# swiss-territorial-data-lab/proj-roadsurf

Hardware: AMD Instinct MI355X
Metric: tiles_per_sec_512x512x3 (higher is better)
Workload: dtype f16 hi + lo operand planes (22 significand bits, 3 MFMA products per product) / f32 accumulate; 1 GPU; Mask R-CNN R50-FPN inference, batch 16 of 512x512 3-band tiles per GPU (BASELINE configs[1]), 800x800 network input; seeded synthetic weights, saturated: 1000 proposals and 100 detections per tile; batch_per_gpu=16, lanes=2, lane_streams=independent, num_classes=2, weights=random

## Files before the change

proj_roadsurf_amd/csrc/bneck_split.hip:

```cpp
#include "conv_tile.h"

namespace {

constexpr int NJ = 2, NT = 256, BM = 4 * NJ * 16, PXW = NJ * 16;

template <int CB, bool PROJ = false>
struct SCfg {
  static constexpr int CBW = 64 * CB;
  static constexpr int C4 = 256 * CB;
  static constexpr int MIB = 4 * CB;
  static constexpr int NPASS = 4 * CB;
  static constexpr int KS2 = 9 * 2 * CB;
  static constexpr int STAGE = (BM + CBW) * 128;
  static constexpr int S3 = 2 * CB + (PROJ ? 2 : 0);
  static constexpr int W3K = CBW + (PROJ ? 64 : 0);
  static constexpr int W3_BYTES = S3 * 64 * 128;
  static constexpr int W1_BYTES = 2 * CBW * 128;
  static constexpr int PASS_BYTES = W3_BYTES + W1_BYTES;
  static constexpr int LDS_BYTES = 2 * STAGE > PASS_BYTES ? 2 * STAGE : PASS_BYTES;
};

__device__ __forceinline__ void split8(const f32x4& a, const f32x4& b, half8& h, half8& l) {
#pragma unroll
  for (int r = 0; r < 4; ++r) {
    const HiLo sa = split_round(a[r]), sb = split_round(b[r]);
    h[r] = sa.h; l[r] = sa.l;
    h[4 + r] = sb.h; l[4 + r] = sb.l;
  }
}
__device__ __forceinline__ float relu_clamp(float v, unsigned& satc, bool count) {
  v = v > 0.f ? v : 0.f;
  satc += count ? rs_sat_bad(v) : 0u;
  return clamp_h16_pos(v);
}

template <int CB, bool NEXT, bool PROJ>
__global__ __launch_bounds__(NT, 2) void bneck_tail_split_kernel(const BneckSplitParams p) {
  using G = SCfg<CB, PROJ>;
  static_assert(!PROJ || CB == 1, "projection form: 64-wide stage only");
  constexpr int CBW = G::CBW, C4 = G::C4, MIB = G::MIB, NPASS = G::NPASS, KS2 = G::KS2, STAGE = G::STAGE;
  extern __shared__ __attribute__((aligned(16))) char smem[];
  const int tid = threadIdx.x, lane = tid & 63;
  const int wave = __builtin_amdgcn_readfirstlane(tid >> 6);
  const int M = p.M;
  const int ntiles = (M + BM - 1) / BM;
  const int q = blockIdx.x;
  if (q >= ntiles) return;
  const int m0 = xcd_tile(q, ntiles) * BM;
  const int lrow = lane >> 3, lchk = lane & 7;
  const half_t* aptr[BM / 32];
#pragma unroll
  for (int ps = 0; ps < BM / 32; ++ps) {
    int m = m0 + ps * 32 + wave * 8 + lrow;
    if (m >= M) m = M - 1;
    const Pix px = pix_of(m, p.W, p.H);
    aptr[ps] = p.t1 + ((long long)(px.n * p.Hp + px.y) * p.Wp + px.x) * CBW + chunk_split(src_chunk(lchk, act_key(lrow)), p.t1_lo);
  }
  const half_t* wptr[CBW / 32];
#pragma unroll
  for (int ps = 0; ps < CBW / 32; ++ps) {
    const int row = ps * 32 + wave * 8 + lrow;
    wptr[ps] = p.w2 + (long long)row * (9 * CBW) + chunk_split(src_chunk(lchk, w_key(row, 4 * MIB)), p.w2_lo);
  }
  auto stage_tap = [&](int buf, int step) {
    char* abase = smem + buf * STAGE;
    const int slice = step / 9, tap = step - slice * 9;
    const int a_off = ((tap / 3) * p.Wp + (tap % 3)) * CBW + slice * 32;
#pragma unroll
    for (int ps = 0; ps < BM / 32; ++ps) glds16(aptr[ps] + a_off, abase + (ps * 32 + wave * 8) * 128);
#pragma unroll
    for (int ps = 0; ps < CBW / 32; ++ps) glds16(wptr[ps] + tap * CBW + slice * 32, abase + BM * 128 + (ps * 32 + wave * 8) * 128);
  };
  auto stage_pass = [&](int pass) {
#pragma unroll
    for (int ps = 0; ps < 2; ++ps) {
      const int row = ps * 32 + wave * 8 + lrow;
      const long long dch = chunk_split(src_chunk(lchk, w_key(row, 16)), p.w3_lo);
#pragma unroll
      for (int s = 0; s < G::S3; ++s)
        glds16(p.w3p + (long long)(pass * 64 + row) * G::W3K + s * 32 + dch, smem + s * 8192 + (ps * 32 + wave * 8) * 128);
    }
    if (NEXT) {
#pragma unroll
      for (int ps = 0; ps < CBW / 32; ++ps) {
        const int row = ps * 32 + wave * 8 + lrow;
        const long long dch = chunk_split(src_chunk(lchk, w_key(row, 4 * MIB)), p.w1_lo);
#pragma unroll
        for (int s = 0; s < 2; ++s)
          glds16(p.w1p + (long long)row * C4 + pass * 64 + s * 32 + dch, smem + G::W3_BYTES + s * CBW * 128 + (ps * 32 + wave * 8) * 128);
      }
    }
  };

  const int fi = lane & 15, fq = lane >> 4, fkey = lane & 7;
  int w_off[4], wB_off[MIB], x_off[NJ];
#pragma unroll
  for (int i = 0; i < 4; ++i) w_off[i] = frag_row(fi, i, 16) * 128;
#pragma unroll
  for (int i = 0; i < MIB; ++i) wB_off[i] = frag_row(fi, i, 4 * MIB) * 128;
#pragma unroll
  for (int j = 0; j < NJ; ++j) x_off[j] = (wave * PXW + j * 16 + fi) * 128;
  const int ch_off = frag_off(fq, fkey, 0), cl_off = frag_off(fq, fkey, 1);

  long long opix[NJ];
  bool valid[NJ];
  unsigned satc = 0;
#pragma unroll
  for (int j = 0; j < NJ; ++j) {
    const int m = m0 + wave * PXW + j * 16 + fi;
    valid[j] = m < M;
    const int mm = valid[j] ? m : M - 1;
    const Pix px = pix_of(mm, p.W, p.H);
    opix[j] = (long long)(px.n * p.Hp + px.y + 1) * p.Wp + px.x + 1;
  }

  f32x4 acc[MIB][NJ];
#pragma unroll
  for (int i = 0; i < MIB; ++i)
#pragma unroll
    for (int j = 0; j < NJ; ++j) acc[i][j] = f32x4{0.f, 0.f, 0.f, 0.f};
  stage_tap(0, 0);
  auto stage_x0 = [&](char* base) {
#pragma unroll
    for (int ps = 0; ps < BM / 32; ++ps) {
      int m = m0 + ps * 32 + wave * 8 + lrow;
      if (m >= M) m = M - 1;
      const Pix px = pix_of(m, p.W, p.H);
      const half_t* xp = p.x0 + ((long long)(px.n * p.Hp + px.y + 1) * p.Wp + px.x + 1) * 64 + chunk_split(src_chunk(lchk, act_key(lrow)), p.x0_lo);
#pragma unroll
      for (int s = 0; s < 2; ++s) glds16(xp + s * 32, base + s * BM * 128 + (ps * 32 + wave * 8) * 128);
    }
  };
  for (int t = 0; t < KS2; ++t) {
    asm volatile("s_waitcnt vmcnt(0)" ::: "memory");
    __syncthreads();
    if (t + 1 < KS2) stage_tap((t + 1) & 1, t + 1);
    const char* sb = smem + (t & 1) * STAGE;
    half8 xh[NJ], xl[NJ];
#pragma unroll
    for (int j = 0; j < NJ; ++j) { xh[j] = *(const half8*)(sb + x_off[j] + ch_off); xl[j] = *(const half8*)(sb + x_off[j] + cl_off); }
#pragma unroll
    for (int i = 0; i < MIB; ++i) {
      const half8 wh = *(const half8*)(sb + BM * 128 + wB_off[i] + ch_off), wl = *(const half8*)(sb + BM * 128 + wB_off[i] + cl_off);
#pragma unroll
      for (int j = 0; j < NJ; ++j) mfma_split3(acc[i][j], wh, wl, xh[j], xl[j]);
    }
  }
  half8 th[2 * CB][NJ], tl[2 * CB][NJ];
  {
#pragma unroll
    for (int i = 0; i < MIB; ++i) {
      const f32x4 sc = *(const f32x4*)(p.s2 + fq * 4 * MIB + i * 4), bv = *(const f32x4*)(p.b2 + fq * 4 * MIB + i * 4);
#pragma unroll
      for (int j = 0; j < NJ; ++j)
#pragma unroll
        for (int r = 0; r < 4; ++r) acc[i][j][r] = relu_clamp(acc[i][j][r] * sc[r] + bv[r], satc, valid[j]);
    }
#pragma unroll
    for (int s = 0; s < 2 * CB; ++s)
#pragma unroll
      for (int j = 0; j < NJ; ++j) split8(acc[2 * s][j], acc[2 * s + 1][j], th[s][j], tl[s][j]);
  }
  half8 x0h[PROJ ? 2 : 1][NJ], x0l[PROJ ? 2 : 1][NJ];
  if (PROJ) {
    const char* xb = smem;
    __syncthreads();
    stage_x0(smem);
    asm volatile("s_waitcnt vmcnt(0)" ::: "memory");
    __syncthreads();
#pragma unroll
    for (int s = 0; s < 2; ++s)
#pragma unroll
      for (int j = 0; j < NJ; ++j) {
        x0h[s][j] = *(const half8*)(xb + s * BM * 128 + x_off[j] + ch_off);
        x0l[s][j] = *(const half8*)(xb + s * BM * 128 + x_off[j] + cl_off);
      }
  }
  f32x4 acc3[MIB][NJ];
#pragma unroll
  for (int i = 0; i < MIB; ++i)
#pragma unroll
    for (int j = 0; j < NJ; ++j) acc3[i][j] = f32x4{0.f, 0.f, 0.f, 0.f};

  for (int pass = 0; pass < NPASS; ++pass) {
    __syncthreads();
    stage_pass(pass);
    const int cb = pass * 64 + fq * 16;
    half8 rh[NJ][2], rl[NJ][2];
    if (!PROJ) {
#pragma unroll
      for (int j = 0; j < NJ; ++j) {
        const half_t* xp = p.x + opix[j] * C4 + cb;
        rh[j][0] = *(const half8*)xp; rh[j][1] = *(const half8*)(xp + 8);
        rl[j][0] = *(const half8*)(xp + p.x_lo); rl[j][1] = *(const half8*)(xp + p.x_lo + 8);
      }
    }
    asm volatile("s_waitcnt vmcnt(0)" ::: "memory");
    __syncthreads();
#pragma unroll
    for (int j = 0; j < NJ; ++j) {
      f32x4 a2[4];
#pragma unroll
      for (int i = 0; i < 4; ++i) {
        a2[i] = f32x4{0.f, 0.f, 0.f, 0.f};
#pragma unroll
        for (int s = 0; s < 2 * CB; ++s) {
          const half8 wh = *(const half8*)(smem + s * 8192 + w_off[i] + ch_off), wl = *(const half8*)(smem + s * 8192 + w_off[i] + cl_off);
          mfma_split3(a2[i], wh, wl, th[s][j], tl[s][j]);
        }
        if (PROJ) {
#pragma unroll
          for (int s = 0; s < 2; ++s) {
            const half8 wh = *(const half8*)(smem + (2 * CB + s) * 8192 + w_off[i] + ch_off), wl = *(const half8*)(smem + (2 * CB + s) * 8192 + w_off[i] + cl_off);
            mfma_split3(a2[i], wh, wl, x0h[s][j], x0l[s][j]);
          }
        }
      }
#pragma unroll
      for (int i = 0; i < 4; ++i) {
        const f32x4 s3v = *(const f32x4*)(p.s3 + cb + i * 4), b3v = *(const f32x4*)(p.b3 + cb + i * 4);
#pragma unroll
        for (int r = 0; r < 4; ++r) {
          const float res = PROJ ? 0.f : (float)rh[j][i >> 1][(i & 1) * 4 + r] + (float)rl[j][i >> 1][(i & 1) * 4 + r];
          a2[i][r] = relu_clamp(a2[i][r] * s3v[r] + b3v[r] + res, satc, valid[j]);
        }
      }
      half8 o0h, o0l, o1h, o1l;
      split8(a2[0], a2[1], o0h, o0l);
      split8(a2[2], a2[3], o1h, o1l);
      if (valid[j]) {
        half_t* op = p.out + opix[j] * C4 + cb;
        *(half8*)op = o0h; *(half8*)(op + 8) = o1h;
        *(half8*)(op + p.out_lo) = o0l; *(half8*)(op + p.out_lo + 8) = o1l;
      }
      if (NEXT) {
#pragma unroll
        for (int i = 0; i < MIB; ++i) {
          const char* wb = smem + G::W3_BYTES + wB_off[i];
          const half8 w0h = *(const half8*)(wb + ch_off), w0l = *(const half8*)(wb + cl_off);
          const half8 w1h = *(const half8*)(wb + CBW * 128 + ch_off), w1l = *(const half8*)(wb + CBW * 128 + cl_off);
          mfma_split3(acc3[i][j], w0h, w0l, o0h, o0l);
          mfma_split3(acc3[i][j], w1h, w1l, o1h, o1l);
        }
      }
    }
  }
  if (NEXT) {
#pragma unroll
    for (int j = 0; j < NJ; ++j) {
      if (!valid[j]) continue;
      half_t* op = p.t1n + opix[j] * CBW + fq * 4 * MIB;
#pragma unroll
      for (int k = 0; k < MIB / 2; ++k) {
        const f32x4 sa = *(const f32x4*)(p.s1 + fq * 4 * MIB + 8 * k), sb2 = *(const f32x4*)(p.s1 + fq * 4 * MIB + 8 * k + 4);
        const f32x4 ba = *(const f32x4*)(p.b1 + fq * 4 * MIB + 8 * k), bb = *(const f32x4*)(p.b1 + fq * 4 * MIB + 8 * k + 4);
        f32x4 va, vb;
#pragma unroll
        for (int r = 0; r < 4; ++r) { va[r] = relu_clamp(acc3[2 * k][j][r] * sa[r] + ba[r], satc, true); vb[r] = relu_clamp(acc3[2 * k + 1][j][r] * sb2[r] + bb[r], satc, true); }
        half8 h, l;
        split8(va, vb, h, l);
        *(half8*)(op + 8 * k) = h;
        *(half8*)(op + p.t1n_lo + 8 * k) = l;
      }
    }
  }
  rs_sat_flush(p.sat, satc);
}

template <int CB, bool PROJ>
int launch_split_cb(const BneckSplitParams& p, hipStream_t stream) {
  using G = SCfg<CB, PROJ>;
  const long long nblk = cdiv(p.M, BM);
  RS_CHECK(nblk < (1ll << 31), RS_ERR_ARG, "bneck_tail_split: grid too large");
  const void* k = p.w1p ? (const void*)bneck_tail_split_kernel<CB, true, PROJ> : (const void*)bneck_tail_split_kernel<CB, false, PROJ>;
  static bool attr[2] = {false, false};
  const int ai = p.w1p ? 1 : 0;
  if (!attr[ai]) {
    RS_HIP(hipFuncSetAttribute(k, hipFuncAttributeMaxDynamicSharedMemorySize, G::LDS_BYTES));
    attr[ai] = true;
  }
  BneckSplitParams pc = p;
  void* args[] = {&pc};
  RS_HIP(hipLaunchKernel(k, dim3((unsigned)nblk), dim3(NT), args, G::LDS_BYTES, stream));
  return RS_OK;
}

}

int launch_bneck_tail_split(const BneckSplitParams& p, hipStream_t stream) {
  RS_CHECK(p.M > 0 && p.t1 && p.w2 && p.b2 && p.s2 && p.w3p && p.b3 && p.s3 && (p.x || p.x0) && !(p.x && p.x0) && p.out, RS_ERR_ARG, "bneck_tail_split: null argument");
  RS_CHECK(p.Hp == p.H + 2 && p.Wp == p.W + 2, RS_ERR_ARG, "bneck_tail_split: maps must carry a halo of 1");
  RS_CHECK(!p.w1p || (p.b1 && p.s1 && p.t1n), RS_ERR_ARG, "bneck_tail_split: next conv1 needs weights, scales, bias and output");
  RS_CHECK(p.CB == 1 || p.CB == 2, RS_ERR_UNSUPPORTED, "bneck_tail_split: bottleneck width %d (64 or 128)", 64 * p.CB);
  if (p.x0) {
    RS_CHECK(p.CB == 1, RS_ERR_UNSUPPORTED, "bneck_tail_split: the projection-shortcut form exists for the 64-wide stage only");
    return launch_split_cb<1, true>(p, stream);
  }
  return p.CB == 1 ? launch_split_cb<1, false>(p, stream) : launch_split_cb<2, false>(p, stream);
}
```

proj_roadsurf_amd/csrc/common.h:

```cpp
#pragma once
#include <hip/hip_runtime.h>
#include <stdint.h>
#include <stdio.h>

typedef _Float16 half_t;
typedef _Float16 half4 __attribute__((ext_vector_type(4)));
typedef _Float16 half8 __attribute__((ext_vector_type(8)));
typedef float f32x4 __attribute__((ext_vector_type(4)));

#define RS_OK 0
#define RS_ERR_ARG -1
#define RS_ERR_HIP -2
#define RS_ERR_BLOB -3
#define RS_ERR_UNSUPPORTED -4

void rs_set_error(const char* fmt, ...);

#define RS_HIP(expr)                                                                       \
  do {                                                                                     \
    hipError_t _e = (expr);                                                                \
    if (_e != hipSuccess) {                                                                \
      rs_set_error("%s:%d: %s -> %s", __FILE__, __LINE__, #expr, hipGetErrorString(_e));   \
      return RS_ERR_HIP;                                                                   \
    }                                                                                      \
  } while (0)

#define RS_CHECK(cond, code, ...)  \
  do {                             \
    if (!(cond)) {                 \
      rs_set_error(__VA_ARGS__);   \
      return (code);               \
    }                              \
  } while (0)

static inline int cdiv(long long a, long long b) { return (int)((a + b - 1) / b); }

#if defined(__HIPCC__)
__device__ __forceinline__ float rs_fdiv(float a, float b) {
  const float y0 = __builtin_amdgcn_rcpf(b);
  const float e = __builtin_fmaf(-b, y0, 1.0f);
  const float y = __builtin_fmaf(e, y0, y0);
  const float q0 = a * y;
  const float r0 = __builtin_fmaf(-b, q0, a);
  const float q1 = __builtin_fmaf(r0, y, q0);
  const float r1 = __builtin_fmaf(-b, q1, a);
  const float q = __builtin_fmaf(r1, y, q1);
  const bool special = !(__builtin_fabsf(b) > 0.f && __builtin_fabsf(b) < __builtin_inff() && __builtin_fabsf(a) > 0.f && __builtin_fabsf(a) < __builtin_inff());
  return special ? a * y0 : q;
}

__device__ __forceinline__ unsigned rs_sat_bad(float f) { return !(__builtin_fabsf(f) <= 65504.f); }
__device__ __forceinline__ void rs_sat_flush(unsigned long long* sat, unsigned cnt) {
  if (sat != nullptr && cnt != 0u) atomicAdd(sat, (unsigned long long)cnt);
}
#endif

struct RsDebug {
  int conv_single_stage_nk = 4;
  int conv_persist = 0;
  int conv_tuned = 1;
  int conv_deep = 1;
  int conv_wide_px = 128;
  int wreg_dbg = 0;
  int wreg_waves = 2;
  int conv_wreg = 1;
  int conv_wide1x1 = 1;
  int stem_small_tile = 1;
  int deep_dbg = 0;
  int deconv_variant = 22;
  int fuse_mask_predictor = 1;
  int side_stream = 1;
  int narrow_roialign = 0;
  int use_glds = 1;
  int fuse_shortcut = 1;
  int fuse_stem = 1;
  int fuse_bneck = 1;
  int deep_tile_px = 1;
  int deep_tail = 1;
  int fuse_rpn_heads = 1;
  int merge_levels = 1;
  int graph_small = 1;
  int use_graph = 0;
  int train_roi_side = -1;
  int train_side = -1;
  int wgrad_target = 512;
  int wgrad_cb = 0;
  int select_debug = 0;
  int nms_debug = 0;
  int roi_window = 1;
  int roi_bwd_atomic = 0;
  int roi_order = 1;
  int poly_edge_cap = 0;
  int poly_vertex_cap = 0;
};
const RsDebug& rs_debug();
void rs_debug_reload();

struct ConvSeg {
  const half_t* in;
  const half_t* w;
  const float* bias;
  void* out;
  float* head_out;
  int Ho, Wo, in_Hp, in_Wp, out_Hp, out_Wp;
  int M;
  int tile0;
  long long in_lo, out_lo;
  const float* wscale;
};
#define RS_MAX_SEGS 5

struct ConvParams {
  const half_t* in;
  const half_t* w;
  const float* bias;
  void* out;
  const half_t* res;
  const half_t* up;
  const int* m_count;
  const int* koff;
  int m_mul;
  int M;
  int Ho, Wo;
  int in_Hp, in_Wp, in_Cs, in_off;
  int stride;
  int KH, KW, Cin;
  int Kpad;
  int Cout;
  int out_Hp, out_Wp, out_Cs, out_pad;
  int up_Hp, up_Wp, up_Cs, up_pad;
  int relu;
  int mode;
  int out_f32;
  const float* dot_w;
  const int* dot_cls;
  const int* dot_slot;
  float* dot_out;
  int dot_k;
  const half_t* in2;
  int in2_Hp, in2_Wp, in2_Cs, in2_off, stride2, Cin2;
  const half_t* down;
  int down_Hp, down_Wp, down_Cs, down_pad;
  const float* res32;
  const half_t* mask;
  int out_stride;
  long long* probe;
  int persist;
  int stages;
  const half_t* head_w;
  const float* head_b;
  float* head_out;
  int nseg;
  int seg_tiles;
  int tail_tiles;
  int split;
  long long in_lo, w_lo, out_lo, res_lo, up_lo, in2_lo;
  const float* wscale;
  long long head_w_lo;
  const float* head_scale;
  ConvSeg seg[RS_MAX_SEGS];
  unsigned long long* sat;
  const unsigned* dy_amax;
  const unsigned* x_amax;
};

int launch_conv(const ConvParams& p, hipStream_t stream, int force_variant , int use_glds);
bool conv_dgrad_split_serves(int rows , int k_channels , int kh, int kw, int stride);
int conv_dgrad_split_variant(const ConvParams& p);
int launch_conv_dgrad_split(const ConvParams& p, hipStream_t stream, int force_variant);
bool conv_fwd_split_serves(int rows , int k_channels , int kh, int kw, int stride);
int conv_fwd_split_variant(const ConvParams& p);
int launch_conv_fwd_split(const ConvParams& p, hipStream_t stream, int force_variant);
int conv_choose_variant(ConvParams& p, int force_variant, int use_glds);
extern thread_local int g_last_conv_variant;

struct StemPoolParams {
  const half_t* in;
  const half_t* wf;
  const float* bias;
  half_t* out;
  int N, in_Hp, in_Wp;
  int Hc, Wc;
  int Hq, Wq;
  unsigned long long* sat;
};
int launch_stem_pool(const StemPoolParams& p, hipStream_t stream);
struct StemPoolSplitParams {
  const half_t* in; long long in_lo;
  const half_t* wf;
  const float* wscale;
  const float* bias;
  half_t* out; long long out_lo;
  int N, in_Hp, in_Wp;
  int Hc, Wc;
  int Hq, Wq;
  unsigned long long* sat;
};
int launch_stem_pool_split(const StemPoolSplitParams& p, hipStream_t stream);

struct BneckParams {
  const half_t* t1;
  const half_t* w2;
  const float* b2;
  const half_t* w3p;
  const float* b3;
  const half_t* x;
  const half_t* x0;
  const half_t* wsc;
  half_t* out;
  const half_t* w1p;
  const float* b1;
  half_t* t1n;
  int M, H, W, Hp, Wp;
  int CB;
  unsigned long long* sat;
};
int launch_bneck_tail(const BneckParams& p, hipStream_t stream);

struct BneckSplitParams {
  const half_t* t1; long long t1_lo;
  const half_t* w2; long long w2_lo;
  const float* b2; const float* s2;
  const half_t* w3p; long long w3_lo;
  const float* b3; const float* s3;
  const half_t* x; long long x_lo;
  half_t* out; long long out_lo;
  const half_t* w1p; long long w1_lo;
  const float* b1; const float* s1;
  half_t* t1n; long long t1n_lo;
  const half_t* x0; long long x0_lo;
  int M, H, W, Hp, Wp;
  int CB;
  unsigned long long* sat;
};
int launch_bneck_tail_split(const BneckSplitParams& p, hipStream_t stream);

int launch_mask_overlap(const uint8_t* det, int n_det, const uint8_t* lab, int n_lab, int h, int w, int* inter, int* lab_area, hipStream_t s);

struct WgradParams {
  const half_t* dy;
  const half_t* x;
  float* partial;
  float* grad;
  const half_t* zeros;
  const float* scale;
  int M, Ho, Wo;
  int dy_Hp, dy_Wp, dy_Cs, dy_pad;
  int in_Hp, in_Wp, in_Cs, in_off;
  int stride, KH, KW, Cin, Cout, Kpad;
  const int* m_count;
  int m_mul;
  int splits;
  int accumulate;
  int f32;
  int split_ops;
  void* split_scratch;
  long long split_dy_cap, split_x_cap;
};
constexpr size_t WGS_ZERO_OFFSET = 128;
constexpr size_t WGS_HEAD_BYTES = 256;
static inline size_t wgrad_split_scratch_bytes(long long dy_cap, long long x_cap) { return WGS_HEAD_BYTES + (size_t)(dy_cap + x_cap) * 4; }
static inline size_t dgrad_split_scratch_bytes(long long cap) { return WGS_HEAD_BYTES + (size_t)cap * 4; }
int launch_dgrad_split_planes(const ConvParams& p, void* scratch, long long cap, hipStream_t stream);
int launch_fwd_split_planes(const ConvParams& p, void* scratch, long long cap, hipStream_t stream);
long long fwd_split_x_elems(const ConvParams& p);
struct SplitRowsDesc {
  const float* w;
  half_t* planes;
  float* inv;
  int rows, k;
  unsigned row_start;
};
int launch_split_rows(const SplitRowsDesc& d, hipStream_t stream);
int launch_split_rows_table(const SplitRowsDesc* table_dev, int n, unsigned total_rows, hipStream_t stream);
bool wgrad_split_serves(const WgradParams& p);
int wgrad_splits(const WgradParams& p);
int launch_conv_wgrad(const WgradParams& p, hipStream_t stream);

struct PreprocParams {
  const uint8_t* tiles;
  half_t* out;
  const int* hb;
  const int* hk;
  const int* vb;
  const int* vk;
  int N, H, W, C;
  int new_h, new_w;
  int out_Hp, out_Wp;
  int ksh, ksv;
  int need_h, need_v;
  int flip;
  int out_f32;
  long long out_lo;
  float mean[4], stdv[4];
  unsigned long long* sat;
};
int launch_preprocess(const PreprocParams& p, hipStream_t s);
int launch_maxpool(const half_t* in, half_t* out, int N, int Hi, int Wi, int Ho, int Wo, int C, hipStream_t s);
int launch_subsample2(const half_t* in, half_t* out, int N, int Hi, int Wi, int Ho, int Wo, int C, hipStream_t s);
int launch_maxpool_f32(const float* in, float* out, int N, int Hi, int Wi, int Ho, int Wo, int C, hipStream_t s);
int launch_maxpool_split(const half_t* in, long long in_lo, half_t* out, long long out_lo, int N, int Hi, int Wi, int Ho, int Wo, int C, hipStream_t s);
int launch_subsample2_split(const half_t* in, long long in_lo, half_t* out, long long out_lo, int N, int Hi, int Wi, int Ho, int Wo, int C, hipStream_t s);
int launch_subsample2_f32(const float* in, float* out, int N, int Hi, int Wi, int Ho, int Wo, int C, hipStream_t s);
int launch_conv_f32(const ConvParams& p, hipStream_t stream, int force_valu = 0, int tile = 0);
int launch_conv_deep(const ConvParams& p, hipStream_t stream, int tile_px = 256);
int rs_device_cu_count();
bool conv_wreg_ok(const ConvParams& p);
int launch_conv_wreg(const ConvParams& p, hipStream_t stream, int waves = 0);
bool conv_wide1x1_split_ok(const ConvParams& p);
int launch_conv_wide1x1_split(const ConvParams& p, hipStream_t stream, int tile_px);
constexpr int WIDE1X1_TILE_PX = 128;
constexpr int WIDE1X1_MIN_M = 4 * 100 * 196;
int launch_conv_deep_multi(const ConvParams& common, const ConvSeg* segs, const int* m_per_image, int nseg, int images, hipStream_t stream);
```

proj_roadsurf_amd/csrc/engine.hip:

```cpp
#include <stdarg.h>
#include <string.h>

#include <cmath>

#include "engine_internal.h"
#include "polygon_pool.h"
#include "train.h"
#include "val_ap.h"

static thread_local char g_err[1024] = "";

static RsDebug g_debug;
static bool g_debug_loaded = false;
void rs_debug_reload() {
  RsDebug d;
  auto rd = [](const char* name, int* v) { const char* e = getenv(name); if (e && *e) *v = atoi(e); };
  rd("RS_CONV_SINGLE_STAGE_NK", &d.conv_single_stage_nk); rd("RS_CONV_PERSIST", &d.conv_persist); rd("RS_CONV_TUNED", &d.conv_tuned);
  rd("RS_CONV_DEEP", &d.conv_deep); rd("RS_CONV_WIDE_PX", &d.conv_wide_px); rd("RS_CONV_WREG", &d.conv_wreg); rd("RS_CONV_WIDE1X1", &d.conv_wide1x1); rd("RS_WREG_DBG", &d.wreg_dbg); rd("RS_ROI_BWD_ATOMIC", &d.roi_bwd_atomic); rd("RS_WREG_WAVES", &d.wreg_waves); rd("RS_STEM_SMALL_TILE", &d.stem_small_tile); rd("RS_DEEP_DBG", &d.deep_dbg);
  rd("RS_DECONV_VARIANT", &d.deconv_variant); rd("RS_FUSE_MASK_PREDICTOR", &d.fuse_mask_predictor); rd("RS_SIDE_STREAM", &d.side_stream);
  rd("RS_NARROW_ROIALIGN", &d.narrow_roialign); rd("RS_USE_GLDS", &d.use_glds); rd("RS_FUSE_SHORTCUT", &d.fuse_shortcut); rd("RS_MERGE_LEVELS", &d.merge_levels); rd("RS_FUSE_RPN_HEADS", &d.fuse_rpn_heads); rd("RS_DEEP_TAIL", &d.deep_tail); rd("RS_DEEP_TILE_PX", &d.deep_tile_px); rd("RS_FUSE_BNECK", &d.fuse_bneck); rd("RS_FUSE_STEM", &d.fuse_stem);
  rd("RS_USE_GRAPH", &d.use_graph); rd("RS_GRAPH_SMALL", &d.graph_small); rd("RS_TRAIN_ROI_SIDE", &d.train_roi_side);
  rd("RS_TRAIN_SIDE", &d.train_side); rd("RS_WGRAD_TARGET", &d.wgrad_target); rd("RS_WGRAD_CB", &d.wgrad_cb);
  rd("RS_SELECT_DEBUG", &d.select_debug); rd("RS_NMS_DEBUG", &d.nms_debug); rd("RS_ROI_WINDOW", &d.roi_window); rd("RS_ROI_ORDER", &d.roi_order);
  rd("RS_POLY_EDGE_CAP", &d.poly_edge_cap); rd("RS_POLY_VERTEX_CAP", &d.poly_vertex_cap);
  g_debug = d;
  g_debug_loaded = true;
}
const RsDebug& rs_debug() {
  if (!g_debug_loaded) rs_debug_reload();
  return g_debug;
}
void rs_set_error(const char* fmt, ...) {
  va_list a;
  va_start(a, fmt);
  vsnprintf(g_err, sizeof g_err, fmt, a);
  va_end(a);
}

extern "C" void rs_resize_shape(int h, int w, int short_edge, int max_size, int* new_h, int* new_w) {
  double scale = (double)short_edge * 1.0 / (double)(h < w ? h : w);
  double newh, neww;
  if (h < w) { newh = short_edge; neww = scale * w; } else { newh = scale * h; neww = short_edge; }
  const double mx = newh > neww ? newh : neww;
  if (mx > max_size) {
    scale = (double)max_size * 1.0 / mx;
    newh = newh * scale;
    neww = neww * scale;
  }
  *new_w = (int)(neww + 0.5);
  *new_h = (int)(newh + 0.5);
}

extern "C" int rs_resize_coeffs(int in_size, int out_size, int32_t* bounds, int32_t* coeffs) {
  const double scale = (double)in_size / (double)out_size;
  const double filterscale = scale < 1.0 ? 1.0 : scale;
  const double support = 1.0 * filterscale;
  const int ksize = (int)ceil(support) * 2 + 1;
  if (!bounds || !coeffs) return ksize;
  const double ss = 1.0 / filterscale;
  std::vector<double> w(ksize);
  for (int xx = 0; xx < out_size; ++xx) {
    const double center = (xx + 0.5) * scale;
    int xmin = (int)(center - support + 0.5);
    if (xmin < 0) xmin = 0;
    int xmax = (int)(center + support + 0.5);
    if (xmax > in_size) xmax = in_size;
    xmax -= xmin;
    double ww = 0.0;
    for (int x = 0; x < ksize; ++x) w[x] = 0.0;
    for (int x = 0; x < xmax; ++x) {
      double a = (x + xmin - center + 0.5) * ss;
      if (a < 0) a = -a;
      const double v = a < 1.0 ? 1.0 - a : 0.0;
      w[x] = v;
      ww += v;
    }
    for (int x = 0; x < xmax; ++x)
      if (ww != 0.0) w[x] /= ww;
    for (int x = 0; x < ksize; ++x) {
      const double v = w[x] * (double)(1 << 22);
      coeffs[xx * ksize + x] = v < 0 ? (int)(v - 0.5) : (int)(v + 0.5);
    }
    bounds[xx * 2] = xmin;
    bounds[xx * 2 + 1] = xmax;
  }
  return ksize;
}

int rs_engine::parse_blob(const void* data, size_t nbytes) {
  const uint8_t* b = (const uint8_t*)data;
  RS_CHECK(nbytes >= 16, RS_ERR_BLOB, "weight blob too small");
  uint32_t hdr[4];
  memcpy(hdr, b, 16);
  RS_CHECK(hdr[0] == 0x52534557u && hdr[1] == 1u, RS_ERR_BLOB, "bad weight blob magic/version %08x/%u", hdr[0], hdr[1]);
  const size_t ent = 96 + 4 + 4 + 32 + 8 + 8;
  RS_CHECK(16 + ent * hdr[2] <= nbytes, RS_ERR_BLOB, "weight blob truncated");
  RS_HIP(hipMalloc(&blob_dev, nbytes));
  RS_HIP(hipMemcpy(blob_dev, data, nbytes, hipMemcpyHostToDevice));
  for (uint32_t i = 0; i < hdr[2]; ++i) {
    const uint8_t* e = b + 16 + ent * i;
    char name[97];
    memcpy(name, e, 96);
    name[96] = 0;
    BlobEntry be;
    uint32_t dt, nd;
    uint64_t dims[4], off, nb;
// ... 1634 lines not shown
```

proj_roadsurf_amd/csrc/ops.hip:

```cpp
#include <string.h>

#include <vector>

#include "../../include/rs_engine.h"
#include "detect.h"
#include "polygon_pool.h"
#include "train.h"
#include "train_stats.h"
#include "val_ap.h"

namespace {

struct OpScratch {
  hipStream_t stream;
  void* held[2] = {nullptr, nullptr};
  int n = 0;
  explicit OpScratch(void* s) : stream((hipStream_t)s) {}
  OpScratch(const OpScratch&) = delete;
  OpScratch& operator=(const OpScratch&) = delete;
  int alloc(void** p, size_t bytes) {
    RS_CHECK(n < 2, RS_ERR_ARG, "OpScratch: more than two buffers");
    RS_HIP(hipMalloc(p, bytes));
    held[n++] = *p;
    return RS_OK;
// ... 107 lines not shown
  if (sa) {
    RS_CHECK(sa->wscale && !in2, RS_ERR_ARG, "split-operand conv: row scales missing (or a second K source, which the operator does not take)");
    p.split = 1; p.in_lo = sa->in_lo; p.w_lo = sa->w_lo; p.out_lo = sa->out_lo; p.res_lo = sa->res_lo; p.up_lo = sa->up_lo; p.wscale = sa->wscale;
  }
  if (in2) {
    RS_CHECK(stride2 >= 1 && (ho - 1) * stride2 < h2 && (wo - 1) * stride2 < w2, RS_ERR_ARG, "second source geometry");
    p.in2 = (const half_t*)in2; p.in2_Hp = h2 + 2 * in2_halo; p.in2_Wp = w2 + 2 * in2_halo; p.in2_Cs = cin2;
    p.in2_off = in2_halo; p.stride2 = stride2; p.Cin2 = cin2;
  }
  OpScratch scratch(stream);
  if (cin < 64 && use_glds >= 0) {
    RS_CHECK(cin == 8, RS_ERR_UNSUPPORTED, "small-Cin path needs cin == 8");
    std::vector<int> koff(kpad / 8, 0);
    for (int t = 0; t < kh * kw && t < (int)koff.size(); ++t) koff[t] = ((t / kw) * p.in_Wp + (t % kw)) * cin;
    int* koff_dev = nullptr;
    { int rc = scratch.alloc((void**)&koff_dev, koff.size() * 4); if (rc) return rc; }
    RS_HIP(hipMemcpy(koff_dev, koff.data(), koff.size() * 4, hipMemcpyHostToDevice));
    p.koff = koff_dev;
  }
  return launch_conv(p, (hipStream_t)stream, variant, use_glds);
}

int rs_debug_set_conv_probe(void* buffer) { g_conv_probe = (long long*)buffer; return RS_OK; }
int rs_op_set_saturation_counter(void* dev_u64) { g_op_sat = (unsigned long long*)dev_u64; return RS_OK; }

int rs_op_conv2d(const void* in, const void* w, const float* bias, void* out, const void* residual, const void* upsample_add,
                 int n, int hi, int wi, int cin, int in_halo, int kh, int kw, int stride, int pad, int cout, int kpad,
                 int out_halo, int relu, int out_f32, int deconv2x, int variant, int use_glds, void* stream) {
  return op_conv2d(in, w, bias, out, residual, upsample_add, n, hi, wi, cin, in_halo, kh, kw, stride, pad, cout, kpad, out_halo,
                   relu, out_f32, deconv2x, variant, use_glds, stream, nullptr, 0, 0, 0, 0, 1);
}

int rs_op_conv2d_split(const void* in, int64_t in_lo, const void* w, int64_t w_lo, const float* wscale, const float* bias, void* out, int64_t out_lo,
                       const void* residual, int64_t res_lo, const void* upsample_add, int64_t up_lo,
                       int n, int hi, int wi, int cin, int in_halo, int kh, int kw, int stride, int pad, int cout, int kpad,
                       int out_halo, int relu, int out_f32, int deconv2x, int variant, void* stream) {
  SplitArgs sa = {in_lo, w_lo, out_lo, res_lo, up_lo, wscale};
  return op_conv2d(in, w, bias, out, residual, upsample_add, n, hi, wi, cin, in_halo, kh, kw, stride, pad, cout, kpad, out_halo,
                   relu, out_f32, deconv2x, variant, 1, stream, nullptr, 0, 0, 0, 0, 1, &sa);
}

int rs_op_deconv_predict_split(const void* in, int64_t in_lo, const void* w, int64_t w_lo, const float* wscale, const float* bias, const float* dot_w, int classes,
                               const int32_t* cls, const int32_t* slot, const int32_t* count_dev, float* logits, int entries, int side, int variant, void* stream) {
  RS_CHECK(in && w && wscale && bias && dot_w && cls && slot && logits && entries > 0 && side > 0 && classes > 0, RS_ERR_ARG, "deconv_predict_split: bad argument");
  ConvParams p;
  memset(&p, 0, sizeof p);
  p.in = (const half_t*)in; p.w = (const half_t*)w; p.bias = bias; p.wscale = wscale;
  p.split = 1; p.in_lo = in_lo; p.w_lo = w_lo;
  p.M = entries * side * side; p.Ho = side; p.Wo = side;
  p.in_Hp = side + 2; p.in_Wp = side + 2; p.in_Cs = 256; p.in_off = 1; p.stride = 1; p.KH = p.KW = 1; p.Cin = 256; p.Kpad = 256; p.Cout = 256;
  p.out_Hp = 2 * side; p.out_Wp = 2 * side; p.out_Cs = 256; p.relu = 1; p.mode = 2;
  p.m_count = count_dev; p.m_mul = side * side;
  p.dot_w = dot_w; p.dot_cls = cls; p.dot_slot = slot; p.dot_out = logits; p.dot_k = classes;
  return launch_conv(p, (hipStream_t)stream, variant, 1);
}

int rs_op_conv2d_dual(const void* in, const void* in2, const void* w, const float* bias, void* out,
                      int n, int hi, int wi, int cin, int in_halo, int kh, int kw, int stride, int pad,
                      int h2, int w2, int cin2, int in2_halo, int stride2,
                      int cout, int kpad, int out_halo, int relu, int variant, void* stream) {
  RS_CHECK(in2, RS_ERR_ARG, "null argument");
  return op_conv2d(in, w, bias, out, nullptr, nullptr, n, hi, wi, cin, in_halo, kh, kw, stride, pad, cout, kpad, out_halo,
                   relu, 0, 0, variant, 1, stream, in2, h2, w2, cin2, in2_halo, stride2);
}

int rs_op_bneck_tail(const void* t1, const void* w2, const float* b2, const void* w3p, const float* b3, const void* x, void* out,
                     const void* w1p, const float* b1, void* t1n, const void* x0, const void* wsc, int n, int h, int w, int width, void* stream) {
  RS_CHECK(t1 && w2 && b2 && w3p && b3 && out && n > 0 && h > 0 && w > 0, RS_ERR_ARG, "bad argument");
  RS_CHECK(width == 64 || width == 128, RS_ERR_UNSUPPORTED, "bneck_tail: bottleneck width %d (64 or 128)", width);
  BneckParams p;
  memset(&p, 0, sizeof p);
  p.t1 = (const half_t*)t1; p.w2 = (const half_t*)w2; p.b2 = b2; p.w3p = (const half_t*)w3p; p.b3 = b3; p.x = (const half_t*)x; p.out = (half_t*)out;
  p.w1p = (const half_t*)w1p; p.b1 = b1; p.t1n = (half_t*)t1n; p.x0 = (const half_t*)x0; p.wsc = (const half_t*)wsc;
  p.M = n * h * w; p.H = h; p.W = w; p.Hp = h + 2; p.Wp = w + 2; p.CB = width / 64;
  p.sat = g_op_sat;
  return launch_bneck_tail(p, (hipStream_t)stream);
}

int rs_op_bneck_tail_split(const void* t1, int64_t t1_lo, const void* w2, const float* s2, const float* b2, const void* w3p, const float* s3, const float* b3,
                           const void* x, int64_t x_lo, void* out, int64_t out_lo, const void* w1p, const float* s1, const float* b1, void* t1n, int64_t t1n_lo,
                           const void* x0, int64_t x0_lo, int n, int h, int w, int width, void* stream) {
  RS_CHECK(t1 && w2 && s2 && b2 && w3p && s3 && b3 && (x || x0) && out && n > 0 && h > 0 && w > 0, RS_ERR_ARG, "bad argument");
  RS_CHECK(width == 64 || width == 128, RS_ERR_UNSUPPORTED, "bneck_tail_split: bottleneck width %d (64 or 128)", width);
  BneckSplitParams p;
  memset(&p, 0, sizeof p);
  p.t1 = (const half_t*)t1; p.t1_lo = t1_lo;
  p.w2 = (const half_t*)w2; p.w2_lo = (long long)width * 9 * width; p.s2 = s2; p.b2 = b2;
  p.w3p = (const half_t*)w3p; p.w3_lo = 4ll * width * (width + (x0 ? 64 : 0)); p.s3 = s3; p.b3 = b3;
  p.x = (const half_t*)x; p.x_lo = x_lo; p.x0 = (const half_t*)x0; p.x0_lo = x0_lo; p.out = (half_t*)out; p.out_lo = out_lo;
  p.w1p = (const half_t*)w1p; p.w1_lo = 4ll * width * width; p.s1 = s1; p.b1 = b1; p.t1n = (half_t*)t1n; p.t1n_lo = t1n_lo;
  p.M = n * h * w; p.H = h; p.W = w; p.Hp = h + 2; p.Wp = w + 2; p.CB = width / 64;
  p.sat = g_op_sat;
  return launch_bneck_tail_split(p, (hipStream_t)stream);
}

int rs_op_mask_overlap(const uint8_t* det_masks, int n_det, const uint8_t* label_masks, int n_labels, int h, int w, int32_t* inter,
                       int32_t* label_area, void* stream) {
  return launch_mask_overlap(det_masks, n_det, label_masks, n_labels, h, w, inter, label_area, (hipStream_t)stream);
}


int rs_op_rasterize_canvas(const double* polys, const int64_t* poly_off, const int32_t* poly_len, const int32_t* inst_first, int n_inst,
                           int side, uint8_t* out) {
  RS_CHECK(inst_first && n_inst >= 0 && (out || n_inst == 0), RS_ERR_ARG, "rasterize_canvas: null table");
  RS_CHECK(side >= 1 && side <= CR_MAX_SIDE, RS_ERR_ARG, "rasterize_canvas: side %d outside [1, %d]", side, CR_MAX_SIDE);
  MtLayout L;
  { int rc = mt_measure(polys, poly_off, poly_len, inst_first, n_inst, 0, &L); if (rc) return rc; }
  RS_CHECK(L.n_doubles <= (size_t)MT_MAX_DOUBLES, RS_ERR_UNSUPPORTED, "rasterize_canvas: more than %d doubles of polygons", MT_MAX_DOUBLES);
  if (n_inst == 0) return RS_OK;
  std::vector<uint8_t> host(L.bytes);
  const int32_t zero = 0;
  mt_pack(host.data(), L, polys, poly_off, poly_len, inst_first, &zero);
  const size_t bytes = (size_t)n_inst * side * ((side + 7) / 8);
  OpScratch scratch(nullptr);
  uint8_t *pool = nullptr, *m = nullptr;
  { int rc = scratch.alloc((void**)&pool, L.bytes); if (rc) return rc; }
  { int rc = scratch.alloc((void**)&m, bytes); if (rc) return rc; }
  RS_HIP(hipMemcpy(pool, host.data(), L.bytes, hipMemcpyHostToDevice));
  CanvasRasterParams q;
  memset(&q, 0, sizeof q);
  q.inst_first = (const int*)(pool + L.o_inst); q.poly_off = (const int*)(pool + L.o_off); q.poly_len = (const int*)(pool + L.o_len);
  q.polys = (const double*)(pool + L.o_xy); q.out = m; q.n_inst = n_inst; q.side = side;
  { int rc = launch_canvas_raster(q, nullptr); if (rc) return rc; }
  RS_HIP(hipMemcpy(out, m, bytes, hipMemcpyDeviceToHost));
  return RS_OK;
}

int rs_op_mask_pair_counts(const uint8_t* det_masks, const int32_t* det_count, int n_tiles, int slots, const uint8_t* gt_masks,
                           const int32_t* tile_first, int gt_cap, int side, int32_t* inter, int32_t* det_area, int32_t* gt_area, void* stream) {
  RS_CHECK(det_masks && det_count && tile_first && inter && det_area && gt_area, RS_ERR_ARG, "mask_pair_counts: null buffer");
  RS_CHECK(side >= 1 && side <= CR_MAX_SIDE, RS_ERR_ARG, "mask_pair_counts: side %d outside [1, %d]", side, CR_MAX_SIDE);
  RS_CHECK(n_tiles >= 1 && slots >= 1 && gt_cap >= 1, RS_ERR_ARG, "mask_pair_counts: %d tiles, %d slots, %d ground truths per tile", n_tiles, slots, gt_cap);
  PairCountParams q;
  memset(&q, 0, sizeof q);
  q.det_masks = det_masks; q.det_count = det_count; q.gt_masks = gt_masks; q.tile_first = tile_first;
  q.inter = inter; q.det_area = det_area; q.gt_area = gt_area; q.n = n_tiles; q.D = slots; q.g_cap = gt_cap;
  q.bytes = (long long)side * ((side + 7) / 8);
  return launch_mask_pair_counts(q, (hipStream_t)stream);
}

static_assert(CM_MAX_CLASSES == RS_MAX_CLASSES && CM_MAX_GT == RS_EVAL_GT_CAP, "coco_match.h restates the header's capacities");
static int coco_match_params(const char* who, CocoMatchParams* q, const float* det_boxes, const float* det_scores, const int32_t* det_classes,
                             const int32_t* det_count, const double* gt_boxes, const int32_t* gt_classes, const int32_t* tile_first,
                             const int32_t* inter, const int32_t* det_area, const int32_t* gt_area, const double* iou_thrs, int n_tiles,
                             int num_classes, int slots, int gt_cap, int32_t* order, int32_t* class_first, int32_t* gt_per_class,
                             uint32_t* matched, uint32_t* ignored, int32_t* npig) {
  RS_CHECK(iou_thrs, RS_ERR_ARG, "%s: null table (the IoU thresholds)", who);
  memset(q, 0, sizeof *q);
  q->det_boxes = det_boxes; q->det_scores = det_scores; q->det_classes = det_classes; q->det_count = det_count;
  q->gt_boxes = gt_boxes; q->gt_classes = gt_classes; q->tile_first = tile_first; q->inter = inter; q->det_area = det_area; q->gt_area = gt_area;
  q->order = order; q->class_first = class_first; q->gt_per_class = gt_per_class; q->matched = matched; q->ignored = ignored; q->npig = npig;
  for (int i = 0; i < CM_THRS; ++i) q->thrs[i] = iou_thrs[i];
  q->n = n_tiles; q->K = num_classes; q->D = slots; q->g_cap = gt_cap;
  return coco_match_check(who, *q);
}
int rs_op_coco_match(const float* det_boxes, const float* det_scores, const int32_t* det_classes, const int32_t* det_count,
                     const double* gt_boxes, const int32_t* gt_classes, const int32_t* tile_first, const int32_t* inter,
                     const int32_t* det_area, const int32_t* gt_area, const double* iou_thrs, int n_tiles, int num_classes, int slots,
                     int gt_cap, int32_t* order, int32_t* class_first, int32_t* gt_per_class, uint32_t* matched, uint32_t* ignored,
                     int32_t* npig, void* stream) {
  CocoMatchParams q;
  { int rc = coco_match_params("rs_op_coco_match", &q, det_boxes, det_scores, det_classes, det_count, gt_boxes, gt_classes, tile_first, inter, det_area,
                               gt_area, iou_thrs, n_tiles, num_classes, slots, gt_cap, order, class_first, gt_per_class, matched, ignored, npig);
    if (rc) return rc; }
  return launch_coco_match(q, (hipStream_t)stream);
}
// ... 647 lines not shown
```

Measured before the change: 959.9 tiles/s.

## Stage a shared row window for bottleneck 3x3 conv taps instead of per-tap tiles

When a tile's output pixels are contiguous in padded row-major order, the bottleneck tail kernel now stages one activation window per (channel slice, kernel row) and reuses it across the three horizontal taps. It indexes that window with per-row offsets. This cuts global-to-LDS activation traffic for the 3x3 conv to about a third, and weights are double-buffered separately. It adds a runtime flag (on by default) with a fallback to the old per-tap staging, plus an asm barrier on pixel offsets to limit register pressure. The window only applies when the tile does not wrap across image rows beyond the window size.

```diff
diff --git a/proj_roadsurf_amd/csrc/bneck_split.hip b/proj_roadsurf_amd/csrc/bneck_split.hip
--- a/proj_roadsurf_amd/csrc/bneck_split.hip
+++ b/proj_roadsurf_amd/csrc/bneck_split.hip
@@ -3,6 +3,7 @@
 namespace {
 
 constexpr int NJ = 2, NT = 256, BM = 4 * NJ * 16, PXW = NJ * 16;
+constexpr int WH = BM + 16;
 
 template <int CB, bool PROJ = false>
 struct SCfg {
@@ -12,12 +13,17 @@
   static constexpr int NPASS = 4 * CB;
   static constexpr int KS2 = 9 * 2 * CB;
   static constexpr int STAGE = (BM + CBW) * 128;
+  static constexpr int WIN = WH * 128;
+  static constexpr int WSLOT = CBW * 128;
+  static constexpr int WIN_BYTES = 2 * WIN + 2 * WSLOT;
   static constexpr int S3 = 2 * CB + (PROJ ? 2 : 0);
   static constexpr int W3K = CBW + (PROJ ? 64 : 0);
   static constexpr int W3_BYTES = S3 * 64 * 128;
   static constexpr int W1_BYTES = 2 * CBW * 128;
   static constexpr int PASS_BYTES = W3_BYTES + W1_BYTES;
-  static constexpr int LDS_BYTES = 2 * STAGE > PASS_BYTES ? 2 * STAGE : PASS_BYTES;
+  static constexpr int CONV2_BYTES = 2 * STAGE > WIN_BYTES ? 2 * STAGE : WIN_BYTES;
+  static constexpr int LDS_BYTES = CONV2_BYTES > PASS_BYTES ? CONV2_BYTES : PASS_BYTES;
+  static_assert(LDS_BYTES <= 80 * 1024, "two workgroups per CU");
 };
 
 __device__ __forceinline__ void split8(const f32x4& a, const f32x4& b, half8& h, half8& l) {
@@ -32,6 +38,11 @@
   v = v > 0.f ? v : 0.f;
   satc += count ? rs_sat_bad(v) : 0u;
   return clamp_h16_pos(v);
+}
+
+__device__ __forceinline__ long long pass_pix(long long opix) {
+  asm volatile("" : "+v"(opix));
+  return opix;
 }
 
 template <int CB, bool NEXT, bool PROJ>
@@ -48,29 +59,17 @@
   if (q >= ntiles) return;
   const int m0 = xcd_tile(q, ntiles) * BM;
   const int lrow = lane >> 3, lchk = lane & 7;
-  const half_t* aptr[BM / 32];
-#pragma unroll
-  for (int ps = 0; ps < BM / 32; ++ps) {
-    int m = m0 + ps * 32 + wave * 8 + lrow;
-    if (m >= M) m = M - 1;
-    const Pix px = pix_of(m, p.W, p.H);
-    aptr[ps] = p.t1 + ((long long)(px.n * p.Hp + px.y) * p.Wp + px.x) * CBW + chunk_split(src_chunk(lchk, act_key(lrow)), p.t1_lo);
-  }
   const half_t* wptr[CBW / 32];
 #pragma unroll
   for (int ps = 0; ps < CBW / 32; ++ps) {
     const int row = ps * 32 + wave * 8 + lrow;
     wptr[ps] = p.w2 + (long long)row * (9 * CBW) + chunk_split(src_chunk(lchk, w_key(row, 4 * MIB)), p.w2_lo);
   }
-  auto stage_tap = [&](int buf, int step) {
-    char* abase = smem + buf * STAGE;
-    const int slice = step / 9, tap = step - slice * 9;
-    const int a_off = ((tap / 3) * p.Wp + (tap % 3)) * CBW + slice * 32;
-#pragma unroll
-    for (int ps = 0; ps < BM / 32; ++ps) glds16(aptr[ps] + a_off, abase + (ps * 32 + wave * 8) * 128);
-#pragma unroll
-    for (int ps = 0; ps < CBW / 32; ++ps) glds16(wptr[ps] + tap * CBW + slice * 32, abase + BM * 128 + (ps * 32 + wave * 8) * 128);
-  };
+  const int mlast = (m0 + BM < M ? m0 + BM : M) - 1;
+  const Pix pfirst = pix_of(m0, p.W, p.H), plast = pix_of(mlast, p.W, p.H);
+  const int c0 = (pfirst.n * p.Hp + pfirst.y) * p.Wp + pfirst.x;
+  const int rlast = (plast.n * p.Hp + plast.y) * p.Wp + plast.x - c0 + 2;
+  const bool window = p.window && rlast < WH;
   auto stage_pass = [&](int pass) {
 #pragma unroll
     for (int ps = 0; ps < 2; ++ps) {
@@ -119,7 +118,6 @@
   for (int i = 0; i < MIB; ++i)
 #pragma unroll
     for (int j = 0; j < NJ; ++j) acc[i][j] = f32x4{0.f, 0.f, 0.f, 0.f};
-  stage_tap(0, 0);
   auto stage_x0 = [&](char* base) {
 #pragma unroll
     for (int ps = 0; ps < BM / 32; ++ps) {
@@ -131,19 +129,90 @@
       for (int s = 0; s < 2; ++s) glds16(xp + s * 32, base + s * BM * 128 + (ps * 32 + wave * 8) * 128);
     }
   };
-  for (int t = 0; t < KS2; ++t) {
-    asm volatile("s_waitcnt vmcnt(0)" ::: "memory");
-    __syncthreads();
-    if (t + 1 < KS2) stage_tap((t + 1) & 1, t + 1);
-    const char* sb = smem + (t & 1) * STAGE;
-    half8 xh[NJ], xl[NJ];
-#pragma unroll
-    for (int j = 0; j < NJ; ++j) { xh[j] = *(const half8*)(sb + x_off[j] + ch_off); xl[j] = *(const half8*)(sb + x_off[j] + cl_off); }
-#pragma unroll
-    for (int i = 0; i < MIB; ++i) {
-      const half8 wh = *(const half8*)(sb + BM * 128 + wB_off[i] + ch_off), wl = *(const half8*)(sb + BM * 128 + wB_off[i] + cl_off);
-#pragma unroll
-      for (int j = 0; j < NJ; ++j) mfma_split3(acc[i][j], wh, wl, xh[j], xl[j]);
+  if (window) {
+    const half_t* wsrc = p.t1 + (long long)c0 * CBW + chunk_split(src_chunk(lchk, act_key(lrow)), p.t1_lo);
+    auto stage_window = [&](int g) {
+      const int slice = g / 3, dy = g - slice * 3;
+      char* wb = smem + (g & 1) * G::WIN;
+      const half_t* src = wsrc + (long long)(dy * p.Wp) * CBW + slice * 32;
+#pragma unroll
+      for (int ps = 0; ps < (WH + 31) / 32; ++ps) {
+        const int r0 = (ps * 4 + wave) * 8;
+        if (ps < WH / 32 || r0 < WH) {
+          const int r = r0 + lrow < rlast ? r0 + lrow : rlast;
+          glds16(src + r * CBW, wb + r0 * 128);
+        }
+      }
+    };
+    auto stage_w2 = [&](int t) {
+      const int slice = t / 9, tap = t - slice * 9;
+      char* wb = smem + 2 * G::WIN + (t & 1) * G::WSLOT;
+#pragma unroll
+      for (int ps = 0; ps < CBW / 32; ++ps) glds16(wptr[ps] + tap * CBW + slice * 32, wb + (ps * 32 + wave * 8) * 128);
+    };
+    int row_of[NJ];
+#pragma unroll
+    for (int j = 0; j < NJ; ++j) row_of[j] = (int)(opix[j] - (p.Wp + 1)) - c0;
+    stage_window(0);
+    stage_w2(0);
+    for (int g = 0; g < KS2 / 3; ++g) {
+      const char* ab = smem + (g & 1) * G::WIN;
+#pragma unroll
+      for (int dx = 0; dx < 3; ++dx) {
+        const int t = g * 3 + dx;
+        asm volatile("s_waitcnt vmcnt(0)" ::: "memory");
+        __syncthreads();
+        if (t + 1 < KS2) stage_w2(t + 1);
+        if (dx == 0 && g + 1 < KS2 / 3) stage_window(g + 1);
+        const char* wsb = smem + 2 * G::WIN + (t & 1) * G::WSLOT;
+        half8 xh[NJ], xl[NJ];
+#pragma unroll
+        for (int j = 0; j < NJ; ++j) {
+          const int r = row_of[j] + dx;
+          xh[j] = *(const half8*)(ab + r * 128 + frag_off(fq, act_key(r), 0));
+          xl[j] = *(const half8*)(ab + r * 128 + frag_off(fq, act_key(r), 1));
+        }
+#pragma unroll
+        for (int i = 0; i < MIB; ++i) {
+          const half8 wh = *(const half8*)(wsb + wB_off[i] + ch_off), wl = *(const half8*)(wsb + wB_off[i] + cl_off);
+#pragma unroll
+          for (int j = 0; j < NJ; ++j) mfma_split3(acc[i][j], wh, wl, xh[j], xl[j]);
+        }
+      }
+    }
+  } else {
+    const half_t* aptr[BM / 32];
+#pragma unroll
+    for (int ps = 0; ps < BM / 32; ++ps) {
+      int m = m0 + ps * 32 + wave * 8 + lrow;
+      if (m >= M) m = M - 1;
+      const Pix px = pix_of(m, p.W, p.H);
+      aptr[ps] = p.t1 + ((long long)(px.n * p.Hp + px.y) * p.Wp + px.x) * CBW + chunk_split(src_chunk(lchk, act_key(lrow)), p.t1_lo);
+    }
+    auto stage_tap = [&](int buf, int step) {
+      char* abase = smem + buf * STAGE;
+      const int slice = step / 9, tap = step - slice * 9;
+      const int a_off = ((tap / 3) * p.Wp + (tap % 3)) * CBW + slice * 32;
+#pragma unroll
+      for (int ps = 0; ps < BM / 32; ++ps) glds16(aptr[ps] + a_off, abase + (ps * 32 + wave * 8) * 128);
+#pragma unroll
+      for (int ps = 0; ps < CBW / 32; ++ps) glds16(wptr[ps] + tap * CBW + slice * 32, abase + BM * 128 + (ps * 32 + wave * 8) * 128);
+    };
+    stage_tap(0, 0);
+    for (int t = 0; t < KS2; ++t) {
+      asm volatile("s_waitcnt vmcnt(0)" ::: "memory");
+      __syncthreads();
+      if (t + 1 < KS2) stage_tap((t + 1) & 1, t + 1);
+      const char* sb = smem + (t & 1) * STAGE;
+      half8 xh[NJ], xl[NJ];
+#pragma unroll
+      for (int j = 0; j < NJ; ++j) { xh[j] = *(const half8*)(sb + x_off[j] + ch_off); xl[j] = *(const half8*)(sb + x_off[j] + cl_off); }
+#pragma unroll
+      for (int i = 0; i < MIB; ++i) {
+        const half8 wh = *(const half8*)(sb + BM * 128 + wB_off[i] + ch_off), wl = *(const half8*)(sb + BM * 128 + wB_off[i] + cl_off);
+#pragma unroll
+        for (int j = 0; j < NJ; ++j) mfma_split3(acc[i][j], wh, wl, xh[j], xl[j]);
+      }
     }
   }
   half8 th[2 * CB][NJ], tl[2 * CB][NJ];
@@ -190,7 +259,7 @@
     if (!PROJ) {
 #pragma unroll
       for (int j = 0; j < NJ; ++j) {
-        const half_t* xp = p.x + opix[j] * C4 + cb;
+        const half_t* xp = p.x + pass_pix(opix[j]) * C4 + cb;
         rh[j][0] = *(const half8*)xp; rh[j][1] = *(const half8*)(xp + 8);
         rl[j][0] = *(const half8*)(xp + p.x_lo); rl[j][1] = *(const half8*)(xp + p.x_lo + 8);
       }
@@ -229,7 +298,7 @@
       split8(a2[0], a2[1], o0h, o0l);
       split8(a2[2], a2[3], o1h, o1l);
       if (valid[j]) {
-        half_t* op = p.out + opix[j] * C4 + cb;
+        half_t* op = p.out + pass_pix(opix[j]) * C4 + cb;
         *(half8*)op = o0h; *(half8*)(op + 8) = o1h;
         *(half8*)(op + p.out_lo) = o0l; *(half8*)(op + p.out_lo + 8) = o1l;
       }
@@ -280,6 +349,7 @@
     attr[ai] = true;
   }
   BneckSplitParams pc = p;
+  pc.window = rs_debug().tail_window != 0;
   void* args[] = {&pc};
   RS_HIP(hipLaunchKernel(k, dim3((unsigned)nblk), dim3(NT), args, G::LDS_BYTES, stream));
   return RS_OK;
diff --git a/proj_roadsurf_amd/csrc/common.h b/proj_roadsurf_amd/csrc/common.h
--- a/proj_roadsurf_amd/csrc/common.h
+++ b/proj_roadsurf_amd/csrc/common.h
@@ -88,6 +88,7 @@
   int select_debug = 0;
   int nms_debug = 0;
   int roi_window = 1;
+  int tail_window = 1;
   int roi_bwd_atomic = 0;
   int roi_order = 1;
   int poly_edge_cap = 0;
@@ -231,6 +232,7 @@
   const half_t* x0; long long x0_lo;
   int M, H, W, Hp, Wp;
   int CB;
+  int window;
   unsigned long long* sat;
 };
 int launch_bneck_tail_split(const BneckSplitParams& p, hipStream_t stream);
diff --git a/proj_roadsurf_amd/csrc/engine.hip b/proj_roadsurf_amd/csrc/engine.hip
--- a/proj_roadsurf_amd/csrc/engine.hip
+++ b/proj_roadsurf_amd/csrc/engine.hip
@@ -21,7 +21,7 @@
   rd("RS_NARROW_ROIALIGN", &d.narrow_roialign); rd("RS_USE_GLDS", &d.use_glds); rd("RS_FUSE_SHORTCUT", &d.fuse_shortcut); rd("RS_MERGE_LEVELS", &d.merge_levels); rd("RS_FUSE_RPN_HEADS", &d.fuse_rpn_heads); rd("RS_DEEP_TAIL", &d.deep_tail); rd("RS_DEEP_TILE_PX", &d.deep_tile_px); rd("RS_FUSE_BNECK", &d.fuse_bneck); rd("RS_FUSE_STEM", &d.fuse_stem);
   rd("RS_USE_GRAPH", &d.use_graph); rd("RS_GRAPH_SMALL", &d.graph_small); rd("RS_TRAIN_ROI_SIDE", &d.train_roi_side);
   rd("RS_TRAIN_SIDE", &d.train_side); rd("RS_WGRAD_TARGET", &d.wgrad_target); rd("RS_WGRAD_CB", &d.wgrad_cb);
-  rd("RS_SELECT_DEBUG", &d.select_debug); rd("RS_NMS_DEBUG", &d.nms_debug); rd("RS_ROI_WINDOW", &d.roi_window); rd("RS_ROI_ORDER", &d.roi_order);
+  rd("RS_SELECT_DEBUG", &d.select_debug); rd("RS_NMS_DEBUG", &d.nms_debug); rd("RS_ROI_WINDOW", &d.roi_window); rd("RS_TAIL_WINDOW", &d.tail_window); rd("RS_ROI_ORDER", &d.roi_order);
   rd("RS_POLY_EDGE_CAP", &d.poly_edge_cap); rd("RS_POLY_VERTEX_CAP", &d.poly_vertex_cap);
   g_debug = d;
   g_debug_loaded = true;
diff --git a/proj_roadsurf_amd/csrc/ops.hip b/proj_roadsurf_amd/csrc/ops.hip
--- a/proj_roadsurf_amd/csrc/ops.hip
+++ b/proj_roadsurf_amd/csrc/ops.hip
@@ -213,6 +213,7 @@
                            const void* x0, int64_t x0_lo, int n, int h, int w, int width, void* stream) {
   RS_CHECK(t1 && w2 && s2 && b2 && w3p && s3 && b3 && (x || x0) && out && n > 0 && h > 0 && w > 0, RS_ERR_ARG, "bad argument");
   RS_CHECK(width == 64 || width == 128, RS_ERR_UNSUPPORTED, "bneck_tail_split: bottleneck width %d (64 or 128)", width);
+  rs_debug_reload();
   BneckSplitParams p;
   memset(&p, 0, sizeof p);
   p.t1 = (const half_t*)t1; p.t1_lo = t1_lo;
```

Result: no change. 968.0 tiles/s (median of 6 runs) (+0.8%).
